# szcompressor/sz

Hardware: AMD Instinct MI355X
Metric: compression GB/s (input), 512^3 float32 ABS 1e-4 (higher is better)
Workload: dtype f32

## Files before the change

sz_amd/csrc/szh_segenc.h:

```cpp
#pragma once

namespace szh_se {
constexpr int NR = 4;
constexpr int INNER = 7;
constexpr int PF = 8;

struct col_t { int b0, b1, s0, s1, o0, o1, rows; };
struct seg_t {
    int bkbeg, bkend, kbeg, kend;
    int nE, E, L;
    int ka, nvec, pitch, kshift;
    int nblk, nruns;
    int lg_nvec;
};
SZH_HD int seg_pitch(int width) { int p = (width + 1) & ~1; if (((p >> 1) & 1) == 0) p += 2; return p; }
SZH_HD col_t make_col(const szh_geom3 &G, int col)
{
    col_t c;
    c.b0 = col / G.g1.num; c.b1 = col - c.b0 * G.g1.num;
    c.s0 = szh_blk_size(G.g0, c.b0); c.s1 = szh_blk_size(G.g1, c.b1); c.o0 = szh_blk_start(G.g0, c.b0); c.o1 = szh_blk_start(G.g1, c.b1);
    c.rows = c.s0 * c.s1;
    return c;
}
SZH_HD seg_t make_seg(const szh_geom3 &G, int rows, int segi, int segb, int VW)
{
    seg_t s;
    s.bkbeg = segi * segb; s.bkend = s.bkbeg + segb < G.g2.num ? s.bkbeg + segb : G.g2.num;
    s.kbeg = szh_blk_start(G.g2, s.bkbeg); s.kend = s.bkend < G.g2.num ? szh_blk_start(G.g2, s.bkend) : G.g2.count;
    s.E = G.g2.early; s.L = G.g2.late;
    int nE = G.g2.split - s.bkbeg; if (nE < 0) nE = 0; if (nE > s.bkend - s.bkbeg) nE = s.bkend - s.bkbeg;
    s.nE = nE;
    s.ka = s.kbeg / VW * VW;
    const int kb = (s.kend + VW - 1) / VW * VW;
    s.nvec = (kb - s.ka) / VW;
    s.pitch = seg_pitch(kb - s.ka); s.kshift = s.kbeg - s.ka;
    s.nblk = s.bkend - s.bkbeg; s.nruns = s.nblk * rows;
    s.lg_nvec = 0; while ((1 << s.lg_nvec) < s.nvec) ++s.lg_nvec;
    return s;
}
inline size_t seg_tile_bytes(const szh_geom3 &G, int segb, int VW)
{
    const size_t rows = (size_t)G.g0.early * G.g1.early;
    const int width = segb * G.g2.early + 2 * VW;
    return (rows * (size_t)seg_pitch(width) * 2 + 15) & ~(size_t)15;
}
inline size_t seg_pieces_per_thread(const szh_geom3 &G, int segb, int VW)
{
    const size_t rows = (size_t)G.g0.early * G.g1.early;
    const size_t nvec = ((size_t)segb * G.g2.early + 2 * VW) / VW + 1;
    size_t p2 = 1; while (p2 < nvec) p2 <<= 1;
    return (rows * p2 + 255) / 256;
}
inline size_t seg_window_words(const szh_geom3 &G, unsigned maxlen) { return (size_t)256 * NR * (size_t)G.g2.early * maxlen / 32 + 8; }
}

#ifdef SZH_HIPSIM
static inline bool any_lane(bool p) { return __ballot(p ? 1 : 0) != 0ull; }
#else
__device__ __forceinline__ bool any_lane(bool p) { return __builtin_amdgcn_ballot_w64(p) != 0ull; }
#endif
__device__ __forceinline__ unsigned magic_of(unsigned d) { return d > 1u ? 0xffffffffu / d + 1u : 0u; }
__device__ __forceinline__ unsigned div_by(unsigned x, unsigned d, unsigned m) { return d > 1u ? (unsigned)(((u64)x * m) >> 32) : x; }

#define SZH_COL_HBINS 256
__global__ __launch_bounds__(256) void k_col_hist(szh_geom3 G, const uint16_t *__restrict__ codes, unsigned nbins, int rshift, int vw, unsigned *__restrict__ col_hist)
{
    SZH_DYN_SMEM(smem);
    unsigned *sh = reinterpret_cast<unsigned *>(smem);
    const unsigned R = 1u << rshift;
    for (unsigned i = threadIdx.x; i < (nbins << rshift); i += 256) sh[i] = 0;
    __syncthreads();
    const szh_se::col_t c = szh_se::make_col(G, (int)blockIdx.x);
    const int nvec = G.g2.count / vw;
    const int lane = (int)threadIdx.x & 63, wid = (int)threadIdx.x >> 6;
    const unsigned rep = threadIdx.x & (R - 1);
    const unsigned m_s1 = magic_of((unsigned)c.s1);
    for (int x = lane; x < nvec; x += 64) {
        for (int r0 = wid; r0 < c.rows; r0 += 16) {
            uint4 w[4];
#pragma unroll
            for (int q = 0; q < 4; ++q) {
                const int r = r0 + 4 * q;
                w[q] = uint4{0u, 0u, 0u, 0u};
                if (r < c.rows) {
                    const int i = (int)div_by((unsigned)r, (unsigned)c.s1, m_s1), j = r - i * c.s1;
                    const uint16_t *src = codes + (int64_t)(c.o0 + i) * G.d0 + (int64_t)(c.o1 + j) * G.d1 + x * vw;
                    if (vw == 8) w[q] = *reinterpret_cast<const uint4 *>(src);
                    else if (vw == 4) { const uint2 t = *reinterpret_cast<const uint2 *>(src); w[q].x = t.x; w[q].y = t.y; }
                    else w[q].x = src[0];
                }
            }
#pragma unroll
            for (int q = 0; q < 4; ++q) {
                if (r0 + 4 * q < c.rows) {
                    const unsigned wv[4] = {w[q].x, w[q].y, w[q].z, w[q].w};
#pragma unroll
                    for (int e = 0; e < 8; ++e) if (e < vw) { const unsigned cd = (e & 1) ? wv[e >> 1] >> 16 : wv[e >> 1] & 0xffffu; atomicAdd(&sh[(cd << rshift) + rep], 1u); }
                }
            }
        }
    }
    __syncthreads();
    for (unsigned b = threadIdx.x; b < nbins; b += 256) {
        unsigned t = 0;
        for (unsigned q = 0; q < R; ++q) t += sh[(b << rshift) + q];
        col_hist[(size_t)blockIdx.x * nbins + b] = t;
// ... 81 lines not shown
    const u64 at = bit0 + (e < nent ? col_bitoff[e] : *total_bits);
    out32[at >> 5] = 0u;
    if (e == nent) out32[(at >> 5) + 1] = 0u;
}
#define SZH_COL_SCAN_PER 8
__global__ __launch_bounds__(1024) void k_col_scan(const u64 *__restrict__ col_bits, const u64 *__restrict__ col_zeros, int nent, u64 *__restrict__ col_bitoff, u64 *__restrict__ col_zoff,
                                                   u64 *total_bits, u64 *total_zeros, u64 bit0, unsigned *out32)
{
    __shared__ u64 shb[16], shz[16];
    const int tid = (int)threadIdx.x, lane = tid & 63, wid = tid >> 6;
    const int lo = tid * SZH_COL_SCAN_PER;
    u64 vb[SZH_COL_SCAN_PER], vz[SZH_COL_SCAN_PER];
#pragma unroll
    for (int q = 0; q < SZH_COL_SCAN_PER; ++q) { const bool in = lo + q < nent; vb[q] = in ? col_bits[lo + q] : 0ull; vz[q] = in ? col_zeros[lo + q] : 0ull; }
    u64 b = 0, z = 0;
#pragma unroll
    for (int q = 0; q < SZH_COL_SCAN_PER; ++q) { b += vb[q]; z += vz[q]; }
    u64 ib = b, iz = z;
    for (int o = 1; o < 64; o <<= 1) { const u64 tb = __shfl_up(ib, o, 64), tz = __shfl_up(iz, o, 64); if (lane >= o) { ib += tb; iz += tz; } }
    if (lane == 63) { shb[wid] = ib; shz[wid] = iz; }
    __syncthreads();
    u64 baseb = 0, basez = 0, totb = 0, totz = 0;
    for (int w = 0; w < 16; ++w) { if (w < wid) { baseb += shb[w]; basez += shz[w]; } totb += shb[w]; totz += shz[w]; }
    u64 rb = baseb + ib - b, rz = basez + iz - z;
#pragma unroll
    for (int q = 0; q < SZH_COL_SCAN_PER; ++q) {
        if (lo + q < nent) { col_bitoff[lo + q] = rb; col_zoff[lo + q] = rz; out32[(bit0 + rb) >> 5] = 0u; }
        rb += vb[q]; rz += vz[q];
    }
    if (tid == 0) { *total_bits = totb; *total_zeros = totz; out32[(bit0 + totb) >> 5] = 0u; out32[((bit0 + totb) >> 5) + 1] = 0u; }
}

__global__ __launch_bounds__(1024) void k_col_zscan(const unsigned *__restrict__ col_zeros, int nent, u64 *__restrict__ col_zoff, u64 *total_zeros)
{
    __shared__ u64 shz[16];
    const int tid = (int)threadIdx.x, lane = tid & 63, wid = tid >> 6;
    const int lo = tid * SZH_COL_SCAN_PER;
    u64 vz[SZH_COL_SCAN_PER], z = 0;
#pragma unroll
    for (int q = 0; q < SZH_COL_SCAN_PER; ++q) { vz[q] = lo + q < nent ? (u64)col_zeros[lo + q] : 0ull; z += vz[q]; }
    u64 iz = z;
    for (int o = 1; o < 64; o <<= 1) { const u64 tz = __shfl_up(iz, o, 64); if (lane >= o) iz += tz; }
    if (lane == 63) shz[wid] = iz;
    __syncthreads();
    u64 basez = 0, totz = 0;
    for (int w = 0; w < 16; ++w) { if (w < wid) basez += shz[w]; totz += shz[w]; }
    u64 rz = basez + iz - z;
#pragma unroll
    for (int q = 0; q < SZH_COL_SCAN_PER; ++q) { if (lo + q < nent) col_zoff[lo + q] = rz; rz += vz[q]; }
    if (tid == 0) *total_zeros = totz;
}

template <class T, bool WIDE>
__global__ __launch_bounds__(256) void k_col_encode(szh_geom3 G, const uint16_t *__restrict__ codes, const u64 *__restrict__ table, unsigned nsym, const szh_se::seg_t *__restrict__ segs, int nseg, int vw,
                                                    size_t tile_bytes, unsigned win_words, const u64 *__restrict__ col_bitoff, const u64 *__restrict__ col_zoff, u64 bit0,
                                                    unsigned *out32, const T *__restrict__ data, T *__restrict__ unpred)
{
    using namespace szh_se;
    SZH_DYN_SMEM(smem);
    __shared__ u64 sh[8];
    __shared__ unsigned rowbase[128];
    u64 *ltab = reinterpret_cast<u64 *>(smem);
    uint16_t *tile = reinterpret_cast<uint16_t *>(smem + ((size_t)nsym + 1) * 8);
    uint16_t *nullrun = reinterpret_cast<uint16_t *>(smem + ((size_t)nsym + 1) * 8 + tile_bytes);
    unsigned *win = reinterpret_cast<unsigned *>(smem + ((size_t)nsym + 1) * 8 + tile_bytes + 16);
    const int tid = (int)threadIdx.x;
    const col_t c = make_col(G, (int)blockIdx.x);
    for (unsigned i = tid; i < nsym; i += 256) ltab[i] = table[i];
    if (tid == 0) ltab[nsym] = 0;
    if (tid < 8) nullrun[tid] = (uint16_t)nsym;
    for (unsigned w = tid; w < win_words; w += 256) win[w] = 0u;
    const unsigned m_rows = magic_of((unsigned)c.rows);
    if (tid < c.rows) { const int i = tid / c.s1, j = tid - i * c.s1; rowbase[tid] = (unsigned)((int64_t)(c.o0 + i) * G.d0 + (int64_t)(c.o1 + j) * G.d1); }
    __syncthreads();
    uint4 pf[PF];
    auto fetch = [&](const seg_t &s) {
        const int lg = s.lg_nvec, mask = (1 << lg) - 1;
#pragma unroll
        for (int p = 0; p < PF; ++p) {
            const int x = p * 256 + tid, r = x >> lg, cv = x & mask;
            pf[p] = uint4{0u, 0u, 0u, 0u};
            if (r < c.rows && cv < s.nvec) {
                const uint16_t *src = codes + (size_t)rowbase[r] + (unsigned)(s.ka + cv * vw);
                if (vw == 8) pf[p] = *reinterpret_cast<const uint4 *>(src);
                else if (vw == 4) { const uint2 t = *reinterpret_cast<const uint2 *>(src); pf[p].x = t.x; pf[p].y = t.y; }
                else pf[p].x = src[0];
            }
        }
    };
    auto place = [&](const seg_t &s) {
        const int lg = s.lg_nvec, mask = (1 << lg) - 1;
        auto put_piece = [&](int r, int cv, const uint4 &w) {
            uint16_t *dst = tile + r * s.pitch + cv * vw;
            if (vw == 8) { unsigned *d = reinterpret_cast<unsigned *>(dst); d[0] = w.x; d[1] = w.y; d[2] = w.z; d[3] = w.w; }
            else if (vw == 4) { unsigned *d = reinterpret_cast<unsigned *>(dst); d[0] = w.x; d[1] = w.y; }
            else dst[0] = (uint16_t)w.x;
        };
#pragma unroll
        for (int p = 0; p < PF; ++p) { const int x = p * 256 + tid, r = x >> lg, cv = x & mask; if (r < c.rows && cv < s.nvec) put_piece(r, cv, pf[p]); }
        for (int x = PF * 256 + tid; (x >> lg) < c.rows; x += 256) {
            const int r = x >> lg, cv = x & mask;
            if (cv >= s.nvec) continue;
            const uint16_t *src = codes + (size_t)rowbase[r] + (unsigned)(s.ka + cv * vw);
            uint4 w = {0u, 0u, 0u, 0u};
            if (vw == 8) w = *reinterpret_cast<const uint4 *>(src);
            else if (vw == 4) { const uint2 t = *reinterpret_cast<const uint2 *>(src); w.x = t.x; w.y = t.y; }
            else w.x = src[0];
            put_piece(r, cv, w);
        }
    };
    seg_t s = segs[0]; s.nruns = s.nblk * c.rows;
    fetch(s);
    const u64 col_bit = bit0 + col_bitoff[blockIdx.x];
    u64 bits_done = 0, zeros_done = col_zoff[blockIdx.x];
    const int null_at = (int)(nullrun - tile);
    for (int segi = 0; segi < nseg; ++segi) {
        place(s);
        __syncthreads();
        seg_t sn = s;
        if (segi + 1 < nseg) { sn = segs[segi + 1]; sn.nruns = sn.nblk * c.rows; fetch(sn); }
        const int nrounds = (s.nruns + 256 * NR - 1) / (256 * NR);
        const int edge_k = s.nE * s.E;
        for (int rd = 0; rd < nrounds; ++rd) {
            const int q0 = (rd * 256 + tid) * NR;
            const int bl0 = (int)div_by((unsigned)q0, (unsigned)c.rows, m_rows), row0 = q0 - bl0 * c.rows;
            unsigned sum1 = 0;
            unsigned elen[WIDE ? NR * INNER : 1], ecode[WIDE ? NR * INNER : 1];
            bool need7[NR];
            if (WIDE) {
                int bl = bl0, row = row0;
#pragma unroll
                for (int j = 0; j < NR; ++j) {
                    const bool on = q0 + j < s.nruns;
                    const int s2 = bl < s.nE ? s.E : s.L, koff = bl < s.nE ? bl * s.E : edge_k + (bl - s.nE) * s.L;
                    const int at = on ? row * s.pitch + s.kshift + koff : null_at;
                    const unsigned *w = reinterpret_cast<const unsigned *>(tile + (at & ~1));
                    unsigned w0 = w[0], w1 = w[1], w2 = w[2], w3 = w[3];
                    if (at & 1) { w0 = (w0 >> 16) | (w1 << 16); w1 = (w1 >> 16) | (w2 << 16); w2 = (w2 >> 16) | (w3 << 16); w3 >>= 16; }
                    const unsigned wv[4] = {w0, w1, w2, w3};
#pragma unroll
                    for (int kk = 0; kk < INNER; ++kk) {
                        unsigned cd = (kk & 1) ? wv[kk >> 1] >> 16 : wv[kk >> 1] & 0xffffu;
                        if (kk == INNER - 1) {
                            cd = (on && s2 == INNER) ? cd : nsym;
                            need7[j] = any_lane(on && s2 == INNER);
                            if (!need7[j]) { elen[j * INNER + kk] = 0u; ecode[j * INNER + kk] = 0u; continue; }
                        }
                        const u64 en = ltab[cd];
                        elen[j * INNER + kk] = (unsigned)en; ecode[j * INNER + kk] = (unsigned)(en >> 32);
                        sum1 += (unsigned)en;
                    }
                    if (++row == c.rows) { row = 0; ++bl; }
                }
            } else {
                int bl = bl0, row = row0;
                for (int j = 0; j < NR; ++j) {
                    if (q0 + j >= s.nruns) break;
                    const int s2 = bl < s.nE ? s.E : s.L, koff = bl < s.nE ? bl * s.E : edge_k + (bl - s.nE) * s.L;
                    const uint16_t *p = tile + row * s.pitch + s.kshift + koff;
                    for (int kk = 0; kk < s2; ++kk) sum1 += (unsigned)ltab[p[kk]];
                    if (++row == c.rows) { row = 0; ++bl; }
                }
            }
            const unsigned bsum = sum1 & 0xffffu, zsum = sum1 >> 16;
            u64 tot2;
            const u64 ex2 = block_excl_scan_256((u64)bsum | ((u64)zsum << 32), sh, &tot2);
            const unsigned tot = (unsigned)tot2, ex = (unsigned)ex2;
            const u64 gbit = col_bit + bits_done;
            const unsigned lead = (unsigned)(gbit & 31u);
            const unsigned nwords = (lead + tot + 31u) >> 5;
            if (bsum) {
                const unsigned bitpos = lead + ex;
                unsigned wpos = bitpos >> 5, nb = bitpos & 31u;
                u64 acc = 0;
                auto put = [&](unsigned le, unsigned cw) {
                    acc = (acc << (le & 63u)) | cw;
                    nb += le & 0xffffu;
                    if (nb >= 32u) { atomicOr(&win[wpos], (unsigned)(acc >> (nb - 32u))); ++wpos; nb -= 32u; }
                };
                if (WIDE) {
#pragma unroll
                    for (int e = 0; e < NR * INNER; ++e) {
                        if (e % INNER == INNER - 1 && !need7[e / INNER]) continue;
                        put(elen[e], ecode[e]);
                    }
                } else {
                    int bl = bl0, row = row0;
                    for (int j = 0; j < NR; ++j) {
                        if (q0 + j >= s.nruns) break;
                        const int s2 = bl < s.nE ? s.E : s.L, koff = bl < s.nE ? bl * s.E : edge_k + (bl - s.nE) * s.L;
                        const uint16_t *p = tile + row * s.pitch + s.kshift + koff;
                        for (int kk = 0; kk < s2; ++kk) { const u64 en = ltab[p[kk]]; put((unsigned)en, (unsigned)(en >> 32)); }
                        if (++row == c.rows) { row = 0; ++bl; }
                    }
                }
                if (nb) atomicOr(&win[wpos], (unsigned)(acc << (32u - nb)));
            }
            if (zsum) {
                u64 zat = zeros_done + (ex2 >> 32);
                int bl = bl0, row = row0;
                for (int j = 0; j < NR; ++j) {
                    if (q0 + j >= s.nruns) break;
                    const int s2 = bl < s.nE ? s.E : s.L, koff = bl < s.nE ? bl * s.E : edge_k + (bl - s.nE) * s.L;
                    const uint16_t *p = tile + row * s.pitch + s.kshift + koff;
                    const T *drow = data + (size_t)rowbase[row] + (unsigned)(s.kbeg + koff);
                    for (int kk = 0; kk < s2; ++kk) if (p[kk] == 0) unpred[zat++] = drow[kk];
                    if (++row == c.rows) { row = 0; ++bl; }
                }
            }
            const bool last_round = rd + 1 == nrounds && segi + 1 == nseg;
            if (tot) {
                __syncthreads();
                const bool partial = ((lead + tot) & 31u) != 0u;
                const unsigned nout = (partial && !last_round) ? nwords - 1 : nwords;
                const u64 w0 = gbit >> 5;
                unsigned keep = 0u;
                if (tid == 0 && partial && !last_round) { keep = win[nwords - 1]; if (nwords > 1) win[nwords - 1] = 0u; }
                for (unsigned w = tid; w < nout; w += 256) {
                    const unsigned x = __builtin_bswap32(win[w]);
                    win[w] = w == 0 ? keep : 0u;
                    const bool shared = (w == 0 && bits_done == 0 && lead != 0u) || (w == nwords - 1 && last_round && partial);
                    if (shared) { if (x) atomicOr(&out32[w0 + w], x); }
                    else out32[w0 + w] = x;
                }
                bits_done += tot;
            } else if (rd + 1 == nrounds && segi + 1 < nseg) __syncthreads();
            zeros_done += tot2 >> 32;
        }
        s = sn;
    }
}

__global__ __launch_bounds__(256) void k_col_zeros(szh_geom3 G, const uint16_t *__restrict__ blk, unsigned *__restrict__ col_zeros)
{
    __shared__ unsigned red[4];
    const szh_se::col_t c = szh_se::make_col(G, (int)blockIdx.x);
    const int64_t base = szh_code_base01(G, c.b0, c.b1), len = (int64_t)c.rows * G.g2.count;
    const int head = (int)(base & 7);
    const int64_t ngroups = (head + len + 7) / 8;
    unsigned z = 0;
    for (int64_t g = threadIdx.x; g < ngroups; g += 256) {
        const uint4 w = *reinterpret_cast<const uint4 *>(blk + (base - head) + g * 8);
        const unsigned wv[4] = {w.x, w.y, w.z, w.w};
#pragma unroll
        for (int e = 0; e < 8; ++e) {
            const int64_t at = g * 8 + e - head;
            const unsigned cd = (e & 1) ? wv[e >> 1] >> 16 : wv[e >> 1] & 0xffffu;
            z += (at >= 0 && at < len && cd == 0u) ? 1u : 0u;
        }
    }
    z = wave_sum_u32(z);
    if ((threadIdx.x & 63) == 0) red[threadIdx.x >> 6] = z;
    __syncthreads();
    if (threadIdx.x == 0) col_zeros[blockIdx.x] = red[0] + red[1] + red[2] + red[3];
}
template <class T>
__global__ __launch_bounds__(256) void k_col_unpack(szh_geom3 G, const uint16_t *__restrict__ blk, uint16_t *__restrict__ nat, const szh_se::seg_t *__restrict__ segs, int nseg, int vw,
                                                    const u64 *__restrict__ col_zoff, const T *__restrict__ unpred, u64 ucap, T *__restrict__ out)
{
    using namespace szh_se;
    SZH_DYN_SMEM(smem);
    __shared__ u64 sh[8];
    __shared__ unsigned rowbase[128];
    uint16_t *L = reinterpret_cast<uint16_t *>(smem);
    const int tid = (int)threadIdx.x;
    const col_t c = make_col(G, (int)blockIdx.x);
    if (tid < c.rows) { const int i = tid / c.s1, j = tid - i * c.s1; rowbase[tid] = (unsigned)((int64_t)(c.o0 + i) * G.d0 + (int64_t)(c.o1 + j) * G.d1); }
    const int64_t col_base = szh_code_base01(G, c.b0, c.b1);
    u64 zeros_done = col_zoff[blockIdx.x];
    for (int segi = 0; segi < nseg; ++segi) {
        const seg_t s = segs[segi];
        const int klen = s.kend - s.kbeg, total = c.rows * klen;
        const int64_t start = col_base + (int64_t)c.rows * s.kbeg;
        const int head = (int)(start & 7), ngroups = (head + total + 7) / 8;
// ... 68 lines not shown
```

sz_amd/csrc/szhip_sz21.inc:

```
template <class T>
int compress_impl(szhip_ctx *ctx, const void *data, int data_on_device, size_t r0, size_t r1, size_t r2, double eb_in,
                  const szhip_params *prm, const unsigned char *meta, size_t meta_len, int out_on_device,
                  unsigned char **out, size_t *out_size, szhip_stats *stats)
{
    const int is_double = sizeof(T) == 8;
    const bool two_d = r0 == 0;
    const szh_geom3 G = two_d ? szh_make_geom2((int)r1, (int)r2) : szh_make_geom3((int)r0, (int)r1, (int)r2);
    const int ncoef = two_d ? 3 : 4;
    const int64_t n = G.n, nb = G.nblocks;
    const T eb = (T)eb_in;
    const double t_begin = now_ms();
    double host_ms = 0;
    const int tp_on = tune_int("SZ_HIP_TIMING", 0); double tp_t[32]; const char *tp_n[32]; int tp_k = 0;
    auto TP = [&](const char *nm) { if (tp_on && tp_k < 32) { tp_t[tp_k] = now_ms() - t_begin; tp_n[tp_k++] = nm; } };
    hipStream_t st = ctx->stream;
    szhip_stats S; memset(&S, 0, sizeof(S));
    S.n_elements = (uint64_t)n; S.n_blocks = (uint64_t)nb;

    const T *d_in = (const T *)data;
    if (!data_on_device) {
        TRY(ensure(ctx, ctx->in, (size_t)n * sizeof(T)));
        TRY(staged_copy(ctx, ctx->in.p, data, (size_t)n * sizeof(T), true));
        d_in = (const T *)ctx->in.p;
    }
// ... 256 lines not shown
            if (ctx->chain_unpred.size() < reg_count * 4 * sizeof(T)) ctx->chain_unpred.resize((reg_count * 4 + reg_count / 4) * sizeof(T));
            for (int e = 0; e < 4; ++e) {
                free(cf.codes[e]); free(cf.unpred[e]);
                cf.codes[e] = ctx->chain_codes.data() + (size_t)e * reg_count;
                cf.unpred[e] = ctx->chain_unpred.data() + (size_t)e * reg_count * sizeof(T);
            }
            join_sections.own = true;
        }
        if (overlap) {
            blk_of_rank.resize(reg_count);
            { size_t r = 0; for (int64_t bb = 0; bb < nb && r < reg_count; ++bb) if (!((ind_bits[bb >> 3] >> (7 - (bb & 7))) & 1)) blk_of_rank[r++] = (uint32_t)bb; if (r != reg_count) FAIL(SZHIP_ERR_INTERNAL, "indicator bits and regression-block count disagree"); }
            for (int e = 0; e < 4; ++e) chain_done[e] = 0;
            for (int e = 0; e < ncoef; ++e)
                section_threads.emplace_back([&, e, chain_in, ind = all_reg_keep.data()] {
                    szhost_coeff_chain_one_p(is_double, chain_in, ind, reg_count, use_mean, e, &cf, &chain_done[e]);
                    make_section(e);
                });
        } else {
            if (!ctx->chain_pool) { ctx->chain_pool = new szhip_chain_pool(); ctx->chain_pool->start(); }
            pool_busy = true;
            for (int e = 0; e < 4; ++e) chain_done[e] = feed && e >= ncoef ? reg_count : 0;
            const size_t *const avail_ptr = two_pieces ? &chain_avail : nullptr;
            ctx->chain_pool->submit(ncoef,
                [&, chain_in, ind = all_reg.data(), avail_ptr](int e) {
                    chain_t0[e] = now_ms() - t_begin;
                    szhost_coeff_chain_one_pa(is_double, chain_in, ind, reg_count, use_mean, e, &cf, feed ? &chain_done[e] : nullptr, avail_ptr);
                    chain_t1[e] = now_ms() - t_begin;
                },
                [&](int e) { make_section(e); });
            if (two_pieces) {
                HIPCHK(hipStreamSynchronize(st));
                __atomic_store_n(&chain_avail, reg_count, __ATOMIC_RELEASE);
            }
            if (!feed) ctx->chain_pool->wait_chains();
        }
        if (!feed) host_ms += now_ms() - h0;
        TP("chain done");
        if (tp_on) fprintf(stderr, "chain threads: %.2f-%.2f %.2f-%.2f %.2f-%.2f %.2f-%.2f | ", chain_t0[0], chain_t1[0], chain_t0[1], chain_t1[1], chain_t0[2], chain_t1[2], chain_t0[3], chain_t1[3]);
        if (!overlap && !feed) {
            HIPCHK(hipMemcpyAsync(ctx->coef_compact.p, hcoef, reg_count * 4 * sizeof(T), hipMemcpyHostToDevice, st));
            hipLaunchKernelGGL((k_move_coef<T, 1>), dim3((unsigned)((nb + 255) / 256)), dim3(256), 0, st, (const uint8_t *)d_lor,
                               (const u64 *)ctx->reg_rank.p, nb, (int64_t)reg_count, d_coef, (T *)ctx->coef_compact.p);
            HIPCHK(hipGetLastError());
        }
    }
    HIPCHK(hipEventRecord(ctx->ev[1], st));
    TP("ev1");

    const bool beam_first = true;
    const bool use_beam = !overlap && beam_first && beam_applies<T>(G, d_in, reg_count);
    const int segenc_sw = tune_int("SZ_HIP_SEGENC", 1);
    bool segenc = !two_d && G.ndim == 3 && segenc_sw != 0 && (!feed || segenc_sw == 2);
    const int se_vw = (G.g2.count % 8) == 0 ? 8 : ((G.g2.count % 4) == 0 ? 4 : 1);
    int se_segb = 0, se_nseg = 0; size_t se_tile = 0;
    if (segenc) {
        bool ok = intervals < 65536;
        const size_t fixed = ((size_t)intervals + 1) * 8 + 16 + szh_se::seg_window_words(G, 32) * 4 + 64;
        const size_t lds_cap = (size_t)63 * 1024, want = (size_t)std::max(4, tune_int("SZ_HIP_SEG_TILE_KB", 24)) * 1024;
        if (ok && fixed + szh_se::seg_tile_bytes(G, 1, se_vw) > lds_cap) ok = false;
        if (ok) {
            const size_t budget = std::min(lds_cap - fixed, std::max(want, szh_se::seg_tile_bytes(G, 1, se_vw)));
            int sb = 1;
            while (sb < G.g2.num && szh_se::seg_tile_bytes(G, sb + 1, se_vw) <= budget && szh_se::seg_pieces_per_thread(G, sb + 1, se_vw) <= (size_t)szh_se::PF) ++sb;
            const int rows_typ = (2 * G.g0.split > G.g0.num ? G.g0.early : G.g0.late) * (2 * G.g1.split > G.g1.num ? G.g1.early : G.g1.late);
            const int per_round = std::max(1, 256 * szh_se::NR / std::max(1, rows_typ));
            if (sb >= per_round) sb = sb / per_round * per_round;
            if (const int f = tune_int("SZ_HIP_SEG_SEGB", 0)) sb = std::max(1, std::min(f, sb));
            se_segb = sb;
            se_nseg = (G.g2.num + se_segb - 1) / se_segb;
            se_tile = szh_se::seg_tile_bytes(G, se_segb, se_vw);
            if ((double)G.g0.num * G.g1.num >= 2.0e9) ok = false;
        }
        segenc = ok;
    }
    int sh_rshift = 0;
    bool seghist = segenc && intervals <= SZH_COL_HBINS && tune_int("SZ_HIP_SEGHIST", 1) != 0;
    if (seghist) { const size_t one = (size_t)intervals * 4; while (sh_rshift < 6 && (one << (sh_rshift + 1)) <= 16 * 1024) ++sh_rshift; }
    const size_t nat_elems = (size_t)n;
    TRY(ensure(ctx, ctx->codes_nat, nat_elems * 2 + 64));
    TRY(ensure(ctx, ctx->codes_blk, (size_t)n * 2 + 64));
    uint16_t *d_nat = (uint16_t *)ctx->codes_nat.p, *d_blk = (uint16_t *)ctx->codes_blk.p;
    int nI, nJ, ntiles;
    using TS = szh_tile_shape<T>;
    TRY(prepare_pencil(ctx, G, szh_gran<T>::NW, TS::TPI, TS::TPJ, &nI, &nJ, &ntiles));
    const int slices_req = tune_int("SZ_HIP_SLICES", ctx->gate ? tune_int("SZ_HIP_SLICES_POOL", 2) : 4);
    const bool sliced = use_beam && slices_req > 1 && !seghist;
    unsigned *tile_done = nullptr;
    const szh_bm::grid_t bgrid = szh_bm::make_grid(G);
    const size_t beam_words = (size_t)bgrid.nKB * bgrid.nJG * szh_bm::WPG;
    if (sliced) {
        const size_t tiles = beam_words;
        TRY(ensure_coherent(ctx, 512 + tiles * 4));
        tile_done = (unsigned *)((char *)ctx->coh + 512);
        if (!ctx->stream3) HIPCHK(hipStreamCreateWithFlags(&ctx->stream3, hipStreamNonBlocking));
        if (!ctx->ev_perm) HIPCHK(hipEventCreateWithFlags(&ctx->ev_perm, hipEventDisableTiming));
    }
    {
        szh_qargs<T> a; memset(&a, 0, sizeof(a));
        a.tile_done = tile_done; a.pub_lines = 32;
        a.G = G; a.data = d_in; a.out = nullptr; a.codes = d_nat; a.blk_lor = d_lor; a.coef = d_coef; a.coef_stride = nb;
        a.eb = eb; a.recip = 1 / eb; a.mean = mean; a.cap = (int)intervals; a.radius = (int)intervals / 2; a.use_mean = use_mean;
        a.faceI = (szh_u64 *)ctx->faceI.p; a.faceJ = (szh_u64 *)ctx->faceJ.p; a.epoch = ++ctx->epoch;
        a.nI = nI; a.nJ = nJ; a.order = (const unsigned *)ctx->order.p; a.no_reg = reg_count == 0;
        a.ticket = (unsigned *)(sm + SM_TICKET); a.err = (unsigned *)(sm + SM_ERR); a.ticket_mode = ctx->ticket_atomic ? 0 : tune_int("SZ_HIP_TICKET_MODE", 2);
        a.progress = (szh_u64 *)ctx->progress.p; a.backoff = SZH_FILL_BACKOFF; a.wide = pencil_wide<T>(G, nJ);
        a.coef_progress = nullptr;
        szh_u64 *coh_prog = nullptr;
        T *dec = nullptr;
        constexpr int64_t LINE = 128 / (int64_t)sizeof(T);
        const int64_t nbp = (nb + LINE - 1) / LINE * LINE;
        if (overlap) {
            TRY(ensure_coherent(ctx, 256));
            TRY(ensure(ctx, ctx->coef_dec, (size_t)nbp * 4 * sizeof(T)));
            coh_prog = (szh_u64 *)ctx->coh;
            dec = (T *)ctx->coef_dec.p;
            a.coef_progress = coh_prog;
            a.coef = dec; a.coef_stride = nbp;
        }
        HIPCHK(hipEventRecord(ctx->ev[2], st));
        if (use_beam) {
            auto feed_slices = [&]() -> int {
                const double h1 = now_ms();
                const int NF = std::max(2, std::min(G.g0.num, 12));
// ... 198 lines not shown
    const u64 total_unpred = h_hist[0];
    S.n_unpred = total_unpred;
    if (!hf) FAIL(SZHIP_ERR_INTERNAL, "Huffman build failed");

    TP("tree built");
    for (auto &x : section_threads) if (x.joinable()) x.join();
    if (pool_busy) { ctx->chain_pool->wait_all(); pool_busy = false; }
    TP("sections joined");
    if (section_failed) { szhost_huff_free(hf); FAIL(SZHIP_ERR_INTERNAL, "coefficient Huffman build failed"); }
    size_t sections_total = 0;
    for (int e = 0; e < ncoef; ++e) sections_total += sec_len[e];
    h0 = now_ms();
    const size_t tree_bytes = szhost_huff_tree_size(hf);
    const size_t pre_len = meta_len + 8 + 4 + sizeof(T) + 4 + 4 + 4 + tree_bytes + 1 + sizeof(T) + ind_bytes;
    const size_t hdr_len = pre_len + sections_total + 8;
    const size_t unpred_bytes = (size_t)total_unpred * sizeof(T);
    const size_t pay_bytes = (size_t)((hf->total_bits + 7) / 8);
    const size_t total_len = hdr_len + unpred_bytes + pay_bytes;
    TRY(ensure_pinned(ctx, pre_len + 8 + 64));
    unsigned char *const hdr = (unsigned char *)ctx->pinned;
    memset(hdr, 0, pre_len + 8);
    {
        unsigned char *q = hdr;
        memcpy(q, meta, meta_len); q += meta_len;
        szhost_put_u64be(q, (uint64_t)n); q += 8;
        szhost_put_u32be(q, (uint32_t)G.block_size); q += 4;
        if (is_double) szhost_put_f64be(q, (double)eb); else szhost_put_f32be(q, (float)eb);
        q += sizeof(T);
        szhost_put_u32be(q, intervals); q += 4;
        szhost_put_u32be(q, (uint32_t)tree_bytes); q += 4;
        szhost_put_u32be(q, (uint32_t)hf->n_nodes); q += 4;
        szhost_huff_tree_write(hf, q); q += tree_bytes;
        *q++ = (unsigned char)use_mean;
        memcpy(q, &mean, sizeof(T)); q += sizeof(T);
        memcpy(q, ind_bits, ind_bytes); q += ind_bytes;
        const uint64_t tu = total_unpred; memcpy(q, &tu, 8); q += 8;
    }
    std::vector<u64> tab_code(intervals); std::vector<uint8_t> tab_len(intervals);
    for (unsigned s = 0; s < intervals; ++s) { tab_code[s] = hf->code[s]; tab_len[s] = hf->len[s]; }
    const u64 total_bits = hf->total_bits;
    szhost_huff_free(hf);
    unsigned enc_maxlen = 0;
    for (unsigned s = 0; s < intervals; ++s) enc_maxlen = std::max<unsigned>(enc_maxlen, tab_len[s]);
    const size_t lds_e32 = (size_t)intervals * 8 + ((size_t)SZH_E32_ROUND * enc_maxlen / 32 + 4) * 4 + 16;
    const bool enc32 = enc_maxlen >= 1 && enc_maxlen <= 32 && lds_e32 <= 60 * 1024 && tune_int("SZ_HIP_ENC32", 1);
    size_t se_lds = 0;
    std::vector<szh_se::seg_t> se_segs;
    if (segenc && enc_maxlen > 32) {
        segenc = false; seghist = false;
        if (sliced) HIPCHK(hipStreamWaitEvent(st, ctx->ev_perm, 0));
        TRY(permute_all());
    }
    if (segenc) {
        se_lds = ((size_t)intervals + 1) * 8 + se_tile + 16 + szh_se::seg_window_words(G, std::max(1u, enc_maxlen)) * 4;
        se_segs.resize((size_t)se_nseg);
        for (int q = 0; q < se_nseg; ++q) se_segs[(size_t)q] = szh_se::make_seg(G, 1, q, se_segb, se_vw);
        TRY(ensure(ctx, ctx->seg_tab, se_segs.size() * sizeof(szh_se::seg_t)));
        HIPCHK(hipMemcpyAsync(ctx->seg_tab.p, se_segs.data(), se_segs.size() * sizeof(szh_se::seg_t), hipMemcpyHostToDevice, st));
    }
    if (segenc) for (unsigned s = 0; s < intervals; ++s) tab_code[s] = (tab_code[s] << 32) | tab_len[s] | (s == 0 ? 0x10000u : 0u);
    else if (enc32) for (unsigned s = 0; s < intervals; ++s) tab_code[s] = (tab_code[s] << 8) | tab_len[s];
    host_ms += now_ms() - h0;

    TRY(ensure(ctx, ctx->code_tab, (size_t)intervals * 8));
    TRY(ensure(ctx, ctx->len_tab, (size_t)intervals));
    HIPCHK(hipMemcpyAsync(ctx->code_tab.p, tab_code.data(), (size_t)intervals * 8, hipMemcpyHostToDevice, st));
    HIPCHK(hipMemcpyAsync(ctx->len_tab.p, tab_len.data(), (size_t)intervals, hipMemcpyHostToDevice, st));
    const bool in_place = out_on_device == 2 && *out && *out_size >= total_len + 64 && ((uintptr_t)*out & 15) == 0 && tune_int("SZ_HIP_OUT_IN_PLACE", 1);
    if (!in_place) TRY(ensure(ctx, ctx->stream_buf, total_len + 64));
    unsigned char *d_stream = in_place ? (unsigned char *)*out : (unsigned char *)ctx->stream_buf.p;
    const int64_t se_nent = (int64_t)ncols;
    if (segenc) {
        TRY(ensure(ctx, ctx->seg_bits, (size_t)se_nent * 8)); TRY(ensure(ctx, ctx->seg_zeros, (size_t)se_nent * 8));
        TRY(ensure(ctx, ctx->seg_bitoff, (size_t)se_nent * 8)); TRY(ensure(ctx, ctx->seg_zoff, (size_t)se_nent * 8));
        const size_t lb = intervals <= 16384 ? (size_t)intervals : 16;
        if (seghist) hipLaunchKernelGGL(k_col_bits_h, dim3((unsigned)((se_nent + 255) / 256)), dim3(256), 0, st, (const unsigned *)ctx->seg_hist.p, (const uint8_t *)ctx->len_tab.p, intervals, se_nent, (u64 *)ctx->seg_bits.p, (u64 *)ctx->seg_zeros.p);
        else
        hipLaunchKernelGGL(k_col_bits, dim3((unsigned)se_nent), dim3(256), lb, st, G, (const uint16_t *)d_nat, (const uint8_t *)ctx->len_tab.p, intervals, se_vw, (u64 *)ctx->seg_bits.p, (u64 *)ctx->seg_zeros.p);
        if (se_nent <= 1024 * SZH_COL_SCAN_PER && tune_int("SZ_HIP_SEG_SCAN1", 1))
            hipLaunchKernelGGL(k_col_scan, dim3(1), dim3(1024), 0, st, (const u64 *)ctx->seg_bits.p, (const u64 *)ctx->seg_zeros.p, (int)se_nent, (u64 *)ctx->seg_bitoff.p, (u64 *)ctx->seg_zoff.p,
                               sm + SM_TOTAL_BITS, sm + SM_TOTAL_UNPRED, (u64)(hdr_len + unpred_bytes) * 8, (unsigned *)d_stream);
        else {
        TRY(scan_u64(ctx, (const u64 *)ctx->seg_bits.p, se_nent, (u64 *)ctx->seg_bitoff.p, sm + SM_TOTAL_BITS));
        TRY(scan_u64(ctx, (const u64 *)ctx->seg_zeros.p, se_nent, (u64 *)ctx->seg_zoff.p, sm + SM_TOTAL_UNPRED));
        hipLaunchKernelGGL(k_col_bounds, dim3((unsigned)((se_nent + 1 + 255) / 256)), dim3(256), 0, st, (const u64 *)ctx->seg_bitoff.p, se_nent, (const u64 *)(sm + SM_TOTAL_BITS),
                           (u64)(hdr_len + unpred_bytes) * 8, (unsigned *)d_stream);
        }
        HIPCHK(hipGetLastError());
    } else
    HIPCHK(hipMemsetAsync(d_stream, 0, total_len + 64, st));
    HIPCHK(hipMemcpyAsync(d_stream, hdr, pre_len, hipMemcpyHostToDevice, st));
    HIPCHK(hipMemcpyAsync(d_stream + pre_len + sections_total, hdr + pre_len, 8, hipMemcpyHostToDevice, st));
    if (sections_total) {
        const hipStream_t ssec = ctx->stream3 ? ctx->stream3 : ctx->stream2;
        HIPCHK(hipEventRecord(ctx->ev_feed, st));
        HIPCHK(hipStreamWaitEvent(ssec, ctx->ev_feed, 0));
        size_t off = pre_len;
        for (int e = 0; e < ncoef; ++e) { HIPCHK(hipMemcpyAsync(d_stream + off, ctx->sec_pin[e], sec_len[e], hipMemcpyHostToDevice, ssec)); off += sec_len[e]; }
        HIPCHK(hipEventRecord(ctx->ev_sec, ssec));
    }
    if (segenc) {
        TRY(ensure(ctx, ctx->unpred, unpred_bytes + 64));
        const unsigned se_win = (unsigned)szh_se::seg_window_words(G, std::max(1u, enc_maxlen));
        if (G.g2.num >= 2 && G.g2.early <= szh_se::INNER && G.g2.late >= szh_se::INNER - 1)
            hipLaunchKernelGGL((k_col_encode<T, true>), dim3((unsigned)se_nent), dim3(256), se_lds, st, G, (const uint16_t *)d_nat, (const u64 *)ctx->code_tab.p, intervals, (const szh_se::seg_t *)ctx->seg_tab.p, se_nseg, se_vw, se_tile, se_win,
                               (const u64 *)ctx->seg_bitoff.p, (const u64 *)ctx->seg_zoff.p, (u64)(hdr_len + unpred_bytes) * 8, (unsigned *)d_stream, d_in, (T *)ctx->unpred.p);
        else
            hipLaunchKernelGGL((k_col_encode<T, false>), dim3((unsigned)se_nent), dim3(256), se_lds, st, G, (const uint16_t *)d_nat, (const u64 *)ctx->code_tab.p, intervals, (const szh_se::seg_t *)ctx->seg_tab.p, se_nseg, se_vw, se_tile, se_win,
                               (const u64 *)ctx->seg_bitoff.p, (const u64 *)ctx->seg_zoff.p, (u64)(hdr_len + unpred_bytes) * 8, (unsigned *)d_stream, d_in, (T *)ctx->unpred.p);
        HIPCHK(hipGetLastError());
        if (total_unpred > 0) HIPCHK(hipMemcpyAsync(d_stream + hdr_len, ctx->unpred.p, unpred_bytes, hipMemcpyDeviceToDevice, st));
    } else {
    if (sliced) HIPCHK(hipStreamWaitEvent(st, ctx->ev_perm, 0));
    if (total_unpred > 0) {
        TRY(ensure(ctx, ctx->unpred, unpred_bytes));
        HIPCHK(hipEventRecord(ctx->ev_in, st));
        HIPCHK(hipStreamWaitEvent(ctx->stream2, ctx->ev_in, 0));
        hipLaunchKernelGGL((k_unpred<T, 0>), dim3(ncols), dim3(256), 0, ctx->stream2, G, (const uint16_t *)d_blk, (const unsigned *)ctx->col_zeros.p,
                           (const u64 *)ctx->col_off.p, d_in, (T *)ctx->unpred.p, (T *)nullptr, (const unsigned *)ctx->zcnt.p,
                           (const unsigned *)ctx->zpos.p, perm_segb, perm_nseg);
        HIPCHK(hipGetLastError());
        HIPCHK(hipEventRecord(ctx->ev_fit, ctx->stream2));
    }
    if (total_bits > 0) {
        const int64_t nchunks = (n + SZH_ENC_CHUNK - 1) / SZH_ENC_CHUNK;
        TRY(ensure(ctx, ctx->chunk_bits, (size_t)nchunks * 8 + 64));
        TRY(ensure(ctx, ctx->chunk_off, (size_t)nchunks * 8));
        hipLaunchKernelGGL(k_chunk_bits, dim3((unsigned)((nchunks + SZH_CB_PER - 1) / SZH_CB_PER)), dim3(256), 0, st, (const uint16_t *)d_blk, n, (const uint8_t *)ctx->len_tab.p,
                           intervals, (u64 *)ctx->chunk_bits.p);
        TRY(scan_u64(ctx, (const u64 *)ctx->chunk_bits.p, nchunks, (u64 *)ctx->chunk_off.p, sm + SM_TOTAL_BITS));
        if (enc32) {
            const int64_t nrounds = (n + SZH_E32_ROUND - 1) / SZH_E32_ROUND;
            hipLaunchKernelGGL(k_encode32, dim3((unsigned)((nrounds + SZH_E32_PER - 1) / SZH_E32_PER)), dim3(256), lds_e32, st, (const uint16_t *)d_blk, n, (const u64 *)ctx->code_tab.p,
                               intervals, (const u64 *)ctx->chunk_off.p, (u64)(hdr_len + unpred_bytes) * 8, (unsigned *)d_stream);
        } else
        hipLaunchKernelGGL(k_encode, dim3((unsigned)((nchunks + SZH_ENC_PER - 1) / SZH_ENC_PER)), dim3(256), 0, st, (const uint16_t *)d_blk, n, (const u64 *)ctx->code_tab.p,
                           (const uint8_t *)ctx->len_tab.p, intervals, (const u64 *)ctx->chunk_off.p, (u64)(hdr_len + unpred_bytes) * 8,
                           (unsigned *)d_stream);
        HIPCHK(hipGetLastError());
    }
    if (total_unpred > 0) {
        HIPCHK(hipStreamWaitEvent(st, ctx->ev_fit, 0));
        HIPCHK(hipMemcpyAsync(d_stream + hdr_len, ctx->unpred.p, unpred_bytes, hipMemcpyDeviceToDevice, st));
    }
    }
    if (sections_total) HIPCHK(hipStreamWaitEvent(st, ctx->ev_sec, 0));
    HIPCHK(hipEventRecord(ctx->ev[4], st));
    TP("encode launched");
    u64 h_small[SM_COUNT];
    HIPCHK(hipMemcpyAsync(h_small, sm, SM_COUNT * 8, hipMemcpyDeviceToHost, st));
    if (out_on_device == 2) {
        if (!*out || *out_size < total_len) FAIL(SZHIP_ERR_ARG, "caller's device buffer too small (%zu < %zu)", *out_size, total_len);
        if (!in_place) HIPCHK(hipMemcpyAsync(*out, d_stream, total_len, hipMemcpyDeviceToDevice, st));
        HIPCHK(hipStreamSynchronize(st));
    } else if (out_on_device) {
        HIPCHK(hipStreamSynchronize(st));
        *out = d_stream;
    } else {
        unsigned char *h = (unsigned char *)malloc(total_len ? total_len : 1);
        if (!h) FAIL(SZHIP_ERR_INTERNAL, "out of host memory");
        TRY(staged_copy(ctx, h, d_stream, total_len, false));
// ... 447 lines not shown
```

Measured before the change: 339.1.

## Recompute Huffman codes in column encoder and size runs per thread dynamically

The column encoder no longer keeps per-run code lengths and codes in register arrays. It sums lengths in a first pass and rereads the tile and table in a second pass to emit bits, which cuts register pressure in exchange for extra LDS reads. The runs-per-thread count is now a runtime value derived from segment size, so the LDS bit window can shrink and rounds balance better. A double-buffered, wave-shuffle scan that skips the zero-count scan when all lanes are zero replaces the generic 256-wide block scan, dropping a barrier. Segment sizing is made even across the column, and the default tile budget is lowered, likely to fit more blocks per CU.

```diff
diff --git a/sz_amd/csrc/szh_segenc.h b/sz_amd/csrc/szh_segenc.h
--- a/sz_amd/csrc/szh_segenc.h
+++ b/sz_amd/csrc/szh_segenc.h
@@ -51,7 +51,7 @@
     size_t p2 = 1; while (p2 < nvec) p2 <<= 1;
     return (rows * p2 + 255) / 256;
 }
-inline size_t seg_window_words(const szh_geom3 &G, unsigned maxlen) { return (size_t)256 * NR * (size_t)G.g2.early * maxlen / 32 + 8; }
+inline size_t seg_window_words(const szh_geom3 &G, unsigned maxlen, int nrmax = NR) { return (size_t)256 * nrmax * (size_t)G.g2.early * maxlen / 32 + 8; }
 }
 
 #ifdef SZH_HIPSIM
@@ -239,19 +239,19 @@
 }
 
 template <class T, bool WIDE>
-__global__ __launch_bounds__(256) void k_col_encode(szh_geom3 G, const uint16_t *__restrict__ codes, const u64 *__restrict__ table, unsigned nsym, const szh_se::seg_t *__restrict__ segs, int nseg, int vw,
+__global__ __launch_bounds__(256) void k_col_encode(szh_geom3 G, const uint16_t *__restrict__ codes, const u64 *__restrict__ table, unsigned nsym, const szh_se::seg_t *__restrict__ segs, int nseg, int vw, int nrmax,
                                                     size_t tile_bytes, unsigned win_words, const u64 *__restrict__ col_bitoff, const u64 *__restrict__ col_zoff, u64 bit0,
                                                     unsigned *out32, const T *__restrict__ data, T *__restrict__ unpred)
 {
     using namespace szh_se;
     SZH_DYN_SMEM(smem);
-    __shared__ u64 sh[8];
+    __shared__ u64 sh[2][4];
     __shared__ unsigned rowbase[128];
     u64 *ltab = reinterpret_cast<u64 *>(smem);
     uint16_t *tile = reinterpret_cast<uint16_t *>(smem + ((size_t)nsym + 1) * 8);
     uint16_t *nullrun = reinterpret_cast<uint16_t *>(smem + ((size_t)nsym + 1) * 8 + tile_bytes);
     unsigned *win = reinterpret_cast<unsigned *>(smem + ((size_t)nsym + 1) * 8 + tile_bytes + 16);
-    const int tid = (int)threadIdx.x;
+    const int tid = (int)threadIdx.x, lane = tid & 63, wid = tid >> 6;
     const col_t c = make_col(G, (int)blockIdx.x);
     for (unsigned i = tid; i < nsym; i += 256) ltab[i] = table[i];
     if (tid == 0) ltab[nsym] = 0;
@@ -299,49 +299,54 @@
     seg_t s = segs[0]; s.nruns = s.nblk * c.rows;
     fetch(s);
     const u64 col_bit = bit0 + col_bitoff[blockIdx.x];
+    const u64 col_word = col_bit >> 5;
+    const bool col_lead = (col_bit & 31u) != 0u;
     u64 bits_done = 0, zeros_done = col_zoff[blockIdx.x];
     const int null_at = (int)(nullrun - tile);
+    int par = 0;
     for (int segi = 0; segi < nseg; ++segi) {
         place(s);
         __syncthreads();
         seg_t sn = s;
         if (segi + 1 < nseg) { sn = segs[segi + 1]; sn.nruns = sn.nblk * c.rows; fetch(sn); }
-        const int nrounds = (s.nruns + 256 * NR - 1) / (256 * NR);
+        const int nrounds = (s.nruns + 256 * nrmax - 1) / (256 * nrmax);
+        const int nr = (s.nruns + 256 * nrounds - 1) / (256 * nrounds);
         const int edge_k = s.nE * s.E;
-        for (int rd = 0; rd < nrounds; ++rd) {
-            const int q0 = (rd * 256 + tid) * NR;
+        auto run_words = [&](int at, unsigned (&wv)[4]) {
+            const unsigned *w = reinterpret_cast<const unsigned *>(tile + (at & ~1));
+            const unsigned w0 = w[0], w1 = w[1], w2 = w[2], w3 = w[3];
+            const unsigned sft = (unsigned)(at & 1) << 4;
+            wv[0] = (unsigned)((((u64)w1 << 32) | w0) >> sft); wv[1] = (unsigned)((((u64)w2 << 32) | w1) >> sft);
+            wv[2] = (unsigned)((((u64)w3 << 32) | w2) >> sft); wv[3] = w3 >> sft;
+        };
+        for (int rd = 0; rd < nrounds; ++rd, par ^= 1) {
+            const int q0 = (rd * 256 + tid) * nr;
             const int bl0 = (int)div_by((unsigned)q0, (unsigned)c.rows, m_rows), row0 = q0 - bl0 * c.rows;
             unsigned sum1 = 0;
-            unsigned elen[WIDE ? NR * INNER : 1], ecode[WIDE ? NR * INNER : 1];
-            bool need7[NR];
+            int jn = 0;
+            unsigned need7 = 0;
             if (WIDE) {
                 int bl = bl0, row = row0;
-#pragma unroll
-                for (int j = 0; j < NR; ++j) {
+                for (int j = 0; j < nr; ++j) {
                     const bool on = q0 + j < s.nruns;
+                    if (!any_lane(on)) break;
+                    jn = j + 1;
                     const int s2 = bl < s.nE ? s.E : s.L, koff = bl < s.nE ? bl * s.E : edge_k + (bl - s.nE) * s.L;
-                    const int at = on ? row * s.pitch + s.kshift + koff : null_at;
-                    const unsigned *w = reinterpret_cast<const unsigned *>(tile + (at & ~1));
-                    unsigned w0 = w[0], w1 = w[1], w2 = w[2], w3 = w[3];
-                    if (at & 1) { w0 = (w0 >> 16) | (w1 << 16); w1 = (w1 >> 16) | (w2 << 16); w2 = (w2 >> 16) | (w3 << 16); w3 >>= 16; }
-                    const unsigned wv[4] = {w0, w1, w2, w3};
+                    unsigned wv[4];
+                    run_words(on ? row * s.pitch + s.kshift + koff : null_at, wv);
+                    const bool n7 = any_lane(on && s2 == INNER);
+                    if (n7) need7 |= 1u << j;
 #pragma unroll
                     for (int kk = 0; kk < INNER; ++kk) {
                         unsigned cd = (kk & 1) ? wv[kk >> 1] >> 16 : wv[kk >> 1] & 0xffffu;
-                        if (kk == INNER - 1) {
-                            cd = (on && s2 == INNER) ? cd : nsym;
-                            need7[j] = any_lane(on && s2 == INNER);
-                            if (!need7[j]) { elen[j * INNER + kk] = 0u; ecode[j * INNER + kk] = 0u; continue; }
-                        }
-                        const u64 en = ltab[cd];
-                        elen[j * INNER + kk] = (unsigned)en; ecode[j * INNER + kk] = (unsigned)(en >> 32);
-                        sum1 += (unsigned)en;
+                        if (kk == INNER - 1) { if (!n7) continue; cd = (on && s2 == INNER) ? cd : nsym; }
+                        sum1 += (unsigned)ltab[cd];
                     }
                     if (++row == c.rows) { row = 0; ++bl; }
                 }
             } else {
                 int bl = bl0, row = row0;
-                for (int j = 0; j < NR; ++j) {
+                for (int j = 0; j < nr; ++j) {
                     if (q0 + j >= s.nruns) break;
                     const int s2 = bl < s.nE ? s.E : s.L, koff = bl < s.nE ? bl * s.E : edge_k + (bl - s.nE) * s.L;
                     const uint16_t *p = tile + row * s.pitch + s.kshift + koff;
@@ -350,13 +355,19 @@
                 }
             }
             const unsigned bsum = sum1 & 0xffffu, zsum = sum1 >> 16;
-            u64 tot2;
-            const u64 ex2 = block_excl_scan_256((u64)bsum | ((u64)zsum << 32), sh, &tot2);
-            const unsigned tot = (unsigned)tot2, ex = (unsigned)ex2;
+            unsigned ib = bsum, iz = zsum;
+            for (int o = 1; o < 64; o <<= 1) { const unsigned t = __shfl_up(ib, o, 64); if (lane >= o) ib += t; }
+            if (any_lane(zsum != 0u)) for (int o = 1; o < 64; o <<= 1) { const unsigned t = __shfl_up(iz, o, 64); if (lane >= o) iz += t; }
+            if (lane == 63) sh[par][wid] = (u64)ib | ((u64)iz << 32);
+            __syncthreads();
+            u64 base2 = 0, tot2 = 0;
+#pragma unroll
+            for (int w = 0; w < 4; ++w) { const u64 t = sh[par][w]; if (w < wid) base2 += t; tot2 += t; }
+            const unsigned tot = (unsigned)tot2, ex = (unsigned)base2 + ib - bsum;
             const u64 gbit = col_bit + bits_done;
             const unsigned lead = (unsigned)(gbit & 31u);
             const unsigned nwords = (lead + tot + 31u) >> 5;
-            if (bsum) {
+            {
                 const unsigned bitpos = lead + ex;
                 unsigned wpos = bitpos >> 5, nb = bitpos & 31u;
                 u64 acc = 0;
@@ -366,14 +377,26 @@
                     if (nb >= 32u) { atomicOr(&win[wpos], (unsigned)(acc >> (nb - 32u))); ++wpos; nb -= 32u; }
                 };
                 if (WIDE) {
-#pragma unroll
-                    for (int e = 0; e < NR * INNER; ++e) {
-                        if (e % INNER == INNER - 1 && !need7[e / INNER]) continue;
-                        put(elen[e], ecode[e]);
+                    int bl = bl0, row = row0;
+                    if (any_lane(bsum != 0u))
+                    for (int j = 0; j < jn; ++j) {
+                        const bool on = q0 + j < s.nruns;
+                        const int s2 = bl < s.nE ? s.E : s.L, koff = bl < s.nE ? bl * s.E : edge_k + (bl - s.nE) * s.L;
+                        unsigned wv[4];
+                        run_words(on ? row * s.pitch + s.kshift + koff : null_at, wv);
+                        const bool n7 = (need7 >> j) & 1u;
+#pragma unroll
+                        for (int kk = 0; kk < INNER; ++kk) {
+                            unsigned cd = (kk & 1) ? wv[kk >> 1] >> 16 : wv[kk >> 1] & 0xffffu;
+                            if (kk == INNER - 1) { if (!n7) continue; cd = (on && s2 == INNER) ? cd : nsym; }
+                            const u64 en = ltab[cd];
+                            put((unsigned)en, (unsigned)(en >> 32));
+                        }
+                        if (++row == c.rows) { row = 0; ++bl; }
                     }
-                } else {
+                } else if (bsum) {
                     int bl = bl0, row = row0;
-                    for (int j = 0; j < NR; ++j) {
+                    for (int j = 0; j < nr; ++j) {
                         if (q0 + j >= s.nruns) break;
                         const int s2 = bl < s.nE ? s.E : s.L, koff = bl < s.nE ? bl * s.E : edge_k + (bl - s.nE) * s.L;
                         const uint16_t *p = tile + row * s.pitch + s.kshift + koff;
@@ -381,12 +404,12 @@
                         if (++row == c.rows) { row = 0; ++bl; }
                     }
                 }
-                if (nb) atomicOr(&win[wpos], (unsigned)(acc << (32u - nb)));
+                if (bsum && nb) atomicOr(&win[wpos], (unsigned)(acc << (32u - nb)));
             }
             if (zsum) {
-                u64 zat = zeros_done + (ex2 >> 32);
+                u64 zat = zeros_done + (unsigned)(base2 >> 32) + iz - zsum;
                 int bl = bl0, row = row0;
-                for (int j = 0; j < NR; ++j) {
+                for (int j = 0; j < nr; ++j) {
                     if (q0 + j >= s.nruns) break;
                     const int s2 = bl < s.nE ? s.E : s.L, koff = bl < s.nE ? bl * s.E : edge_k + (bl - s.nE) * s.L;
                     const uint16_t *p = tile + row * s.pitch + s.kshift + koff;
@@ -406,7 +429,7 @@
                 for (unsigned w = tid; w < nout; w += 256) {
                     const unsigned x = __builtin_bswap32(win[w]);
                     win[w] = w == 0 ? keep : 0u;
-                    const bool shared = (w == 0 && bits_done == 0 && lead != 0u) || (w == nwords - 1 && last_round && partial);
+                    const bool shared = (col_lead && w0 + w == col_word) || (w == nwords - 1 && last_round && partial);
                     if (shared) { if (x) atomicOr(&out32[w0 + w], x); }
                     else out32[w0 + w] = x;
                 }
diff --git a/sz_amd/csrc/szhip_sz21.inc b/sz_amd/csrc/szhip_sz21.inc
--- a/sz_amd/csrc/szhip_sz21.inc
+++ b/sz_amd/csrc/szhip_sz21.inc
@@ -332,23 +332,25 @@
     const int segenc_sw = tune_int("SZ_HIP_SEGENC", 1);
     bool segenc = !two_d && G.ndim == 3 && segenc_sw != 0 && (!feed || segenc_sw == 2);
     const int se_vw = (G.g2.count % 8) == 0 ? 8 : ((G.g2.count % 4) == 0 ? 4 : 1);
-    int se_segb = 0, se_nseg = 0; size_t se_tile = 0;
+    int se_segb = 0, se_nseg = 0, se_nrmax = szh_se::NR; size_t se_tile = 0;
     if (segenc) {
-        bool ok = intervals < 65536;
+        bool ok = intervals < 65536 && (double)n < 4.0e9;
+        if ((int64_t)G.g0.late * G.g1.late * G.g2.late < 32) ok = false;
         const size_t fixed = ((size_t)intervals + 1) * 8 + 16 + szh_se::seg_window_words(G, 32) * 4 + 64;
-        const size_t lds_cap = (size_t)63 * 1024, want = (size_t)std::max(4, tune_int("SZ_HIP_SEG_TILE_KB", 24)) * 1024;
+        const size_t lds_cap = (size_t)63 * 1024, want = (size_t)std::max(4, tune_int("SZ_HIP_SEG_TILE_KB", 14)) * 1024;
         if (ok && fixed + szh_se::seg_tile_bytes(G, 1, se_vw) > lds_cap) ok = false;
         if (ok) {
             const size_t budget = std::min(lds_cap - fixed, std::max(want, szh_se::seg_tile_bytes(G, 1, se_vw)));
             int sb = 1;
             while (sb < G.g2.num && szh_se::seg_tile_bytes(G, sb + 1, se_vw) <= budget && szh_se::seg_pieces_per_thread(G, sb + 1, se_vw) <= (size_t)szh_se::PF) ++sb;
-            const int rows_typ = (2 * G.g0.split > G.g0.num ? G.g0.early : G.g0.late) * (2 * G.g1.split > G.g1.num ? G.g1.early : G.g1.late);
-            const int per_round = std::max(1, 256 * szh_se::NR / std::max(1, rows_typ));
-            if (sb >= per_round) sb = sb / per_round * per_round;
+            sb = (G.g2.num + (G.g2.num + sb - 1) / sb - 1) / ((G.g2.num + sb - 1) / sb);
             if (const int f = tune_int("SZ_HIP_SEG_SEGB", 0)) sb = std::max(1, std::min(f, sb));
             se_segb = sb;
             se_nseg = (G.g2.num + se_segb - 1) / se_segb;
             se_tile = szh_se::seg_tile_bytes(G, se_segb, se_vw);
+            const int rows_typ = (2 * G.g0.split > G.g0.num ? G.g0.early : G.g0.late) * (2 * G.g1.split > G.g1.num ? G.g1.early : G.g1.late);
+            const int runs_typ = std::max(1, sb * rows_typ), rounds_typ = (runs_typ + 256 * szh_se::NR - 1) / (256 * szh_se::NR);
+            se_nrmax = std::max(1, std::min(szh_se::NR, (runs_typ + 256 * rounds_typ - 1) / (256 * rounds_typ)));
             if ((double)G.g0.num * G.g1.num >= 2.0e9) ok = false;
         }
         segenc = ok;
@@ -653,7 +655,7 @@
         TRY(permute_all());
     }
     if (segenc) {
-        se_lds = ((size_t)intervals + 1) * 8 + se_tile + 16 + szh_se::seg_window_words(G, std::max(1u, enc_maxlen)) * 4;
+        se_lds = ((size_t)intervals + 1) * 8 + se_tile + 16 + szh_se::seg_window_words(G, std::max(1u, enc_maxlen), se_nrmax) * 4;
         se_segs.resize((size_t)se_nseg);
         for (int q = 0; q < se_nseg; ++q) se_segs[(size_t)q] = szh_se::make_seg(G, 1, q, se_segb, se_vw);
         TRY(ensure(ctx, ctx->seg_tab, se_segs.size() * sizeof(szh_se::seg_t)));
@@ -702,12 +704,12 @@
     }
     if (segenc) {
         TRY(ensure(ctx, ctx->unpred, unpred_bytes + 64));
-        const unsigned se_win = (unsigned)szh_se::seg_window_words(G, std::max(1u, enc_maxlen));
+        const unsigned se_win = (unsigned)szh_se::seg_window_words(G, std::max(1u, enc_maxlen), se_nrmax);
         if (G.g2.num >= 2 && G.g2.early <= szh_se::INNER && G.g2.late >= szh_se::INNER - 1)
-            hipLaunchKernelGGL((k_col_encode<T, true>), dim3((unsigned)se_nent), dim3(256), se_lds, st, G, (const uint16_t *)d_nat, (const u64 *)ctx->code_tab.p, intervals, (const szh_se::seg_t *)ctx->seg_tab.p, se_nseg, se_vw, se_tile, se_win,
+            hipLaunchKernelGGL((k_col_encode<T, true>), dim3((unsigned)se_nent), dim3(256), se_lds, st, G, (const uint16_t *)d_nat, (const u64 *)ctx->code_tab.p, intervals, (const szh_se::seg_t *)ctx->seg_tab.p, se_nseg, se_vw, se_nrmax, se_tile, se_win,
                                (const u64 *)ctx->seg_bitoff.p, (const u64 *)ctx->seg_zoff.p, (u64)(hdr_len + unpred_bytes) * 8, (unsigned *)d_stream, d_in, (T *)ctx->unpred.p);
         else
-            hipLaunchKernelGGL((k_col_encode<T, false>), dim3((unsigned)se_nent), dim3(256), se_lds, st, G, (const uint16_t *)d_nat, (const u64 *)ctx->code_tab.p, intervals, (const szh_se::seg_t *)ctx->seg_tab.p, se_nseg, se_vw, se_tile, se_win,
+            hipLaunchKernelGGL((k_col_encode<T, false>), dim3((unsigned)se_nent), dim3(256), se_lds, st, G, (const uint16_t *)d_nat, (const u64 *)ctx->code_tab.p, intervals, (const szh_se::seg_t *)ctx->seg_tab.p, se_nseg, se_vw, se_nrmax, se_tile, se_win,
                                (const u64 *)ctx->seg_bitoff.p, (const u64 *)ctx->seg_zoff.p, (u64)(hdr_len + unpred_bytes) * 8, (unsigned *)d_stream, d_in, (T *)ctx->unpred.p);
         HIPCHK(hipGetLastError());
         if (total_unpred > 0) HIPCHK(hipMemcpyAsync(d_stream + hdr_len, ctx->unpred.p, unpred_bytes, hipMemcpyDeviceToDevice, st));
```

After: 375.8 (median of 6 runs). +10.8%, better.
